# blue-yonder/tsfresh

Measured on AMD Instinct MI355X. Metric: series/sec (ComprehensiveFCParameters, len=1024), higher is better.
Workload: dtype f64; 1 GPU; 100000 series/GPU x len 1024 float32 i.i.d. N(0,1), ComprehensiveFCParameters (783 columns), inputs and outputs resident in HBM; n_series_per_gpu=100000, length=1024, n_cols=783, parallelism=ids1

## Files before the change

tsfresh_amd/csrc/fam_spectral.h:

```cpp
#ifndef TSFA_FAM_SPECTRAL_H
#define TSFA_FAM_SPECTRAL_H

#include "tsfa_common.h"

#define TSFA_TW_N 65536

TSFA_DEV bool is_pow2(int n) { return n > 0 && (n & (n - 1)) == 0; }

TSFA_DEV void blk_fft_stages_dit(const Blk &b, double *re, double *im, int M, const double *twc, const double *tws);

TSFA_DEV void blk_fft_pow2(const Blk &b, double *re, double *im, int M, const double *twc, const double *tws) {
    int logM = 0;
    while ((1 << logM) < M) ++logM;
    blk_sync();
    for (int i = b.tid; i < M; i += b.nt) {
#if TSFA_GPU
        const int j = (logM > 0) ? (int)(__builtin_bitreverse32((unsigned)i) >> (32 - logM)) : 0;
#else
        unsigned r = 0, x = (unsigned)i;
        for (int k = 0; k < logM; ++k) {
            r = (r << 1) | (x & 1u);
            x >>= 1;
        }
        const int j = (int)r;
#endif
        if (j > i) {
            const double tr = re[i], ti = im[i];
            re[i] = re[j];
            im[i] = im[j];
            re[j] = tr;
            im[j] = ti;
        }
    }
    blk_fft_stages_dit(b, re, im, M, twc, tws);
}

TSFA_DEV void blk_fft_stages_dit(const Blk &b, double *re, double *im, int M, const double *twc, const double *tws) {
    int logM = 0;
    while ((1 << logM) < M) ++logM;
    int st = 0;
    if (logM & 1) {
        blk_sync();
        for (int t = b.tid; t < (M >> 1); t += b.nt) {
            const int i0 = 2 * t, i1 = i0 + 1;
            const double wr = twc[0], wi = tws[0];
            const double xr = re[i1], xi = im[i1];
            const double tr = xr * wr - xi * wi;
            const double ti = xr * wi + xi * wr;
            const double ur = re[i0], ui = im[i0];
            re[i1] = ur - tr;
            im[i1] = ui - ti;
            re[i0] = ur + tr;
            im[i0] = ui + ti;
        }
        st = 1;
    }
    for (; st + 1 < logM; st += 2) {
        const int h = 1 << st;
        const int strideA = TSFA_TW_N / (2 * h), strideB = TSFA_TW_N / (4 * h);
        blk_sync();
        for (int t = b.tid; t < (M >> 2); t += b.nt) {
            const int grp = t >> st, k = t & (h - 1);
            const int i0 = grp * 4 * h + k, i1 = i0 + h, i2 = i0 + 2 * h, i3 = i0 + 3 * h;
            const double war = twc[k * strideA], wai = tws[k * strideA];
            const double wbr0 = twc[k * strideB], wbi0 = tws[k * strideB];
            const double wbr1 = twc[(k + h) * strideB], wbi1 = tws[(k + h) * strideB];
            const double x0r = re[i0], x0i = im[i0], x1r = re[i1], x1i = im[i1];
            const double x2r = re[i2], x2i = im[i2], x3r = re[i3], x3i = im[i3];
            double tr = x1r * war - x1i * wai, ti = x1r * wai + x1i * war;
            const double a1r = x0r - tr, a1i = x0i - ti, a0r = x0r + tr, a0i = x0i + ti;
            tr = x3r * war - x3i * wai;
            ti = x3r * wai + x3i * war;
            const double a3r = x2r - tr, a3i = x2i - ti, a2r = x2r + tr, a2i = x2i + ti;
            tr = a2r * wbr0 - a2i * wbi0;
            ti = a2r * wbi0 + a2i * wbr0;
            re[i2] = a0r - tr;
            im[i2] = a0i - ti;
            re[i0] = a0r + tr;
            im[i0] = a0i + ti;
            tr = a3r * wbr1 - a3i * wbi1;
            ti = a3r * wbi1 + a3i * wbr1;
            re[i3] = a1r - tr;
            im[i3] = a1i - ti;
            re[i1] = a1r + tr;
            im[i1] = a1i + ti;
        }
    }
    blk_sync();
}

TSFA_DEV void blk_fft_pow2_batch(const Blk &b, double *re, double *im, int M, int nb, const double *twc, const double *tws) {
    int logM = 0;
    while ((1 << logM) < M) ++logM;
    blk_sync();
    for (int ii = b.tid; ii < nb * M; ii += b.nt) {
        const int base = ii & ~(M - 1), i = ii & (M - 1);
#if TSFA_GPU
        const int j = (logM > 0) ? (int)(__builtin_bitreverse32((unsigned)i) >> (32 - logM)) : 0;
#else
        unsigned r = 0, x = (unsigned)i;
        for (int k = 0; k < logM; ++k) {
            r = (r << 1) | (x & 1u);
            x >>= 1;
        }
        const int j = (int)r;
#endif
        if (j > i) {
            const double tr = re[base + i], ti = im[base + i];
            re[base + i] = re[base + j];
            im[base + i] = im[base + j];
            re[base + j] = tr;
            im[base + j] = ti;
        }
    }
    int st = 0;
    if (logM & 1) {
        blk_sync();
        for (int t = b.tid; t < nb * (M >> 1); t += b.nt) {
            const int i0 = 2 * t, i1 = i0 + 1;
            const double wr = twc[0], wi = tws[0];
            const double xr = re[i1], xi = im[i1];
            const double tr = xr * wr - xi * wi;
            const double ti = xr * wi + xi * wr;
            const double ur = re[i0], ui = im[i0];
            re[i1] = ur - tr;
            im[i1] = ui - ti;
            re[i0] = ur + tr;
            im[i0] = ui + ti;
        }
        st = 1;
    }
    const int lq = logM - 2;
    for (; st + 1 < logM; st += 2) {
        const int h = 1 << st;
        const int strideA = TSFA_TW_N / (2 * h), strideB = TSFA_TW_N / (4 * h);
        blk_sync();
        for (int tt = b.tid; tt < nb * (M >> 2); tt += b.nt) {
            const int blk = tt >> lq, t = tt & ((M >> 2) - 1);
            const int grp = t >> st, k = t & (h - 1);
            const int i0 = blk * M + grp * 4 * h + k, i1 = i0 + h, i2 = i0 + 2 * h, i3 = i0 + 3 * h;
            const double war = twc[k * strideA], wai = tws[k * strideA];
            const double wbr0 = twc[k * strideB], wbi0 = tws[k * strideB];
            const double wbr1 = twc[(k + h) * strideB], wbi1 = tws[(k + h) * strideB];
            const double x0r = re[i0], x0i = im[i0], x1r = re[i1], x1i = im[i1];
            const double x2r = re[i2], x2i = im[i2], x3r = re[i3], x3i = im[i3];
            double tr = x1r * war - x1i * wai, ti = x1r * wai + x1i * war;
            const double a1r = x0r - tr, a1i = x0i - ti, a0r = x0r + tr, a0i = x0i + ti;
            tr = x3r * war - x3i * wai;
            ti = x3r * wai + x3i * war;
            const double a3r = x2r - tr, a3i = x2i - ti, a2r = x2r + tr, a2i = x2i + ti;
            tr = a2r * wbr0 - a2i * wbi0;
            ti = a2r * wbi0 + a2i * wbr0;
            re[i2] = a0r - tr;
            im[i2] = a0i - ti;
            re[i0] = a0r + tr;
            im[i0] = a0i + ti;
            tr = a3r * wbr1 - a3i * wbi1;
            ti = a3r * wbi1 + a3i * wbr1;
            re[i3] = a1r - tr;
            im[i3] = a1i - ti;
            re[i1] = a1r + tr;
            im[i1] = a1i + ti;
        }
    }
    blk_sync();
}

#define TSFA_GOERTZEL_MIN 257

template <class G>
TSFA_DEV void blk_rfft(const Blk &b, int n, G g, double *Xr, double *Xi, double *tc, double *ts,
                       const double *twc, const double *tws) {
    const int nh = n / 2;
    if (is_pow2(n) && n >= 4 && n <= TSFA_TW_N) {
        const int M = nh;
        blk_sync();
        for (int k = b.tid; k < M; k += b.nt) {
            Xr[k] = g(2 * k);
            Xi[k] = g(2 * k + 1);
        }
        blk_fft_pow2(b, Xr, Xi, M, twc, tws);
        const int stride = TSFA_TW_N / n;
        for (int k = b.tid; k <= M / 2; k += b.nt) {
            if (k == 0) {
                const double zr = Xr[0], zi = Xi[0];
                Xr[0] = zr + zi;
                Xi[0] = 0.0;
                Xr[M] = zr - zi;
                Xi[M] = 0.0;
            } else {
                const int k2 = M - k;
                const double ar = Xr[k], ai = Xi[k], br = Xr[k2], bi = Xi[k2];
                {
                    const double er = 0.5 * (ar + br), ei = 0.5 * (ai - bi);
                    const double orr = 0.5 * (ai + bi), oi = -0.5 * (ar - br);
                    const double wr = twc[k * stride], wi = tws[k * stride];
                    Xr[k] = er + (orr * wr - oi * wi);
                    Xi[k] = ei + (orr * wi + oi * wr);
                }
                if (k2 != k) {
                    const double er = 0.5 * (br + ar), ei = 0.5 * (bi - ai);
                    const double orr = 0.5 * (bi + ai), oi = -0.5 * (br - ar);
                    const double wr = twc[k2 * stride], wi = tws[k2 * stride];
                    Xr[k2] = er + (orr * wr - oi * wi);
                    Xi[k2] = ei + (orr * wi + oi * wr);
                }
            }
        }
        blk_sync();
        return;
    }
    double x_first;
    {
        double acc = 0.0;
        for (int j = b.tid; j < n; j += b.nt) acc += g(j);
        x_first = blk_sum(b, acc) / (double)n;
        if (!(x_first == x_first) || isinf(x_first)) x_first = 0.0;
    }
    if (n > 32768) {
        blk_sync();
        for (int k0 = 4 * b.tid; k0 <= nh; k0 += 4 * b.nt) {
            double kap[4], sg[4], sn[4], cs[4], s1[4], d1[4];
#pragma unroll
            for (int u = 0; u < 4; ++u) {
                double sh, ch;
                tsfa_sincospi(2.0 * (double)(k0 + u) / (double)n, &sn[u], &cs[u]);
                tsfa_sincospi((double)(k0 + u) / (double)n, &sh, &ch);
                const bool pos = cs[u] >= 0.0;
                kap[u] = pos ? -4.0 * sh * sh : 4.0 * ch * ch;
                sg[u] = pos ? 1.0 : -1.0;
                s1[u] = 0.0;
                d1[u] = 0.0;
            }
            for (int j = 0; j < n; ++j) {
                const double x = g(j) - x_first;
#pragma unroll
                for (int u = 0; u < 4; ++u) {
                    const double d = (x + kap[u] * s1[u]) + sg[u] * d1[u];
                    s1[u] = sg[u] * s1[u] + d;
                    d1[u] = d;
                }
            }
#pragma unroll
            for (int u = 0; u < 4; ++u) {
                const int k = k0 + u;
                if (k > nh) continue;
                Xr[k] = 0.5 * kap[u] * s1[u] + sg[u] * d1[u] + ((k == 0) ? (double)n * x_first : 0.0);
                Xi[k] = (k == 0 || 2 * k == n) ? 0.0 : s1[u] * sn[u];
            }
        }
        blk_sync();
        return;
    }
    if (n >= TSFA_GOERTZEL_MIN) {
        blk_sync();
        for (int k0 = 4 * b.tid; k0 <= nh; k0 += 4 * b.nt) {
            double c[4], sn[4], cs[4], s1[4], s2[4];
#pragma unroll
            for (int u = 0; u < 4; ++u) {
                tsfa_sincospi(2.0 * (double)(k0 + u) / (double)n, &sn[u], &cs[u]);
                c[u] = 2.0 * cs[u];
                s1[u] = 0.0;
                s2[u] = 0.0;
            }
            for (int j = 0; j < n; ++j) {
                const double x = g(j) - x_first;
#pragma unroll
                for (int u = 0; u < 4; ++u) {
                    const double s0 = (x + c[u] * s1[u]) - s2[u];
                    s2[u] = s1[u];
                    s1[u] = s0;
                }
            }
#pragma unroll
            for (int u = 0; u < 4; ++u) {
                const int k = k0 + u;
                if (k > nh) continue;
                Xr[k] = s1[u] * cs[u] - s2[u] + ((k == 0) ? (double)n * x_first : 0.0);
                Xi[k] = (k == 0 || 2 * k == n) ? 0.0 : s1[u] * sn[u];
            }
        }
        blk_sync();
        return;
    }
    blk_sync();
    for (int j = b.tid; j < n; j += b.nt) {
        double s, c;
        tsfa_sincospi(2.0 * (double)j / (double)n, &s, &c);
        tc[j] = c;
        ts[j] = -s;
    }
    blk_sync_all();
    for (int k = b.tid; k <= nh; k += b.nt) {
        double ar = 0.0, ai = 0.0;
        int idx = 0;
        for (int j = 0; j < n; ++j) {
            const double x = g(j) - x_first;
            ar += x * tc[idx];
            ai += x * ts[idx];
            idx += k;
            if (idx >= n) idx -= n;
        }
        if (k == 0 || (2 * k == n)) ai = 0.0;
        if (k == 0) ar += (double)n * x_first;
        Xr[k] = ar;
        Xi[k] = ai;
    }
    blk_sync();
}

#define TSFA_BLUESTEIN_MAXM 65536

TSFA_DEV int tsfa_bitrev(int i, int bits) {
#if TSFA_GPU
    return (bits > 0) ? (int)(__builtin_bitreverse32((unsigned)i) >> (32 - bits)) : 0;
#else
    unsigned r = 0, x = (unsigned)i;
    for (int k = 0; k < bits; ++k) { r = (r << 1) | (x & 1u); x >>= 1; }
    return (int)r;
#endif
}

TSFA_DEV void blk_fft_stages_dif(const Blk &b, double *re, double *im, int M, const double *twc, const double *tws) {
    int logM = 0;
    while ((1 << logM) < M) ++logM;
    int st = logM;
    for (; st >= 2; st -= 2) {
        const int h = 1 << (st - 2);
        const int strideA = TSFA_TW_N / (4 * h), strideB = TSFA_TW_N / (2 * h);
        blk_sync();
        for (int t = b.tid; t < (M >> 2); t += b.nt) {
            const int grp = t >> (st - 2), k = t & (h - 1);
            const int i0 = grp * 4 * h + k, i1 = i0 + h, i2 = i0 + 2 * h, i3 = i0 + 3 * h;
            const double wa0r = twc[k * strideA], wa0i = tws[k * strideA];
            const double wa1r = twc[(k + h) * strideA], wa1i = tws[(k + h) * strideA];
            const double wbr = twc[k * strideB], wbi = tws[k * strideB];
            const double x0r = re[i0], x0i = im[i0], x1r = re[i1], x1i = im[i1];
            const double x2r = re[i2], x2i = im[i2], x3r = re[i3], x3i = im[i3];
            const double a0r = x0r + x2r, a0i = x0i + x2i, d0r = x0r - x2r, d0i = x0i - x2i;
            const double a2r = d0r * wa0r - d0i * wa0i, a2i = d0r * wa0i + d0i * wa0r;
            const double a1r = x1r + x3r, a1i = x1i + x3i, d1r = x1r - x3r, d1i = x1i - x3i;
// ... 208 lines not shown
                Xi[N] = 0.0;
            } else {
                const int k2 = N - k;
                double ar, ai, br, bi;
                zbin(k, &ar, &ai);
                zbin(k2, &br, &bi);
                {
                    const double er = 0.5 * (ar + br), ei = 0.5 * (ai - bi);
                    const double orr = 0.5 * (ai + bi), oi = -0.5 * (ar - br);
                    double c, s;
                    unit(2 * k, &c, &s);
                    const double wr = c, wi = -s;
                    Xr[k] = er + (orr * wr - oi * wi);
                    Xi[k] = ei + (orr * wi + oi * wr);
                }
                if (k2 != k) {
                    const double er = 0.5 * (br + ar), ei = 0.5 * (bi - ai);
                    const double orr = 0.5 * (bi + ai), oi = -0.5 * (br - ar);
                    double c, s;
                    unit(2 * k2, &c, &s);
                    const double wr = c, wi = -s;
                    Xr[k2] = er + (orr * wr - oi * wi);
                    Xi[k2] = ei + (orr * wi + oi * wr);
                }
            }
        }
    }
    blk_sync();
}

template <class ST>
TSFA_DEV int blk_welch(const Blk &b, const ST *xs, int n, double *win, double *pxx, double *Xr, double *Xi,
                       double *tc, double *ts, const double *twc, const double *tws, int xcap = 0,
                       const double *hann256 = nullptr) {
    const int nper = (n < 256) ? n : 256;
    const int nover = nper / 2;
    const int step = nper - nover;
    const int nseg = (n - nover) / step;
    const int nf = nper / 2 + 1;
    blk_sync();
    double w2 = 0.0;
    for (int j = b.tid; j < nper; j += b.nt) {
        double wv;
        if (nper == 256 && hann256 != nullptr) wv = hann256[j];
        else {
            const double fac = np_linspace_at(-M_PI, M_PI, nper + 1, j);
            wv = (nper <= 1) ? 1.0 : (0.5 + 0.5 * cos(fac));
        }
        win[j] = wv;
        w2 += wv * wv;
    }
    for (int k = b.tid; k < nf; k += b.nt) pxx[k] = 0.0;
    w2 = blk_sum(b, w2);
    const double scale = 1.0 / w2;
    const int nbmax = (xcap / 128 < TSFA_RED_DOUBLES / 2) ? xcap / 128 : TSFA_RED_DOUBLES / 2;
    if (nper == 256 && nseg > 1 && nbmax >= 2) {
        const int M = 128;
        const int stride_tw = TSFA_TW_N / 256;
        for (int s0 = 0; s0 < nseg; s0 += nbmax) {
            const int nb = (nseg - s0 < nbmax) ? (nseg - s0) : nbmax;
            blk_sync();
#if TSFA_GPU
            {
                const int lane = b.tid & 63, wave = b.tid >> 6, nwav = (b.nt + 63) >> 6;
                for (int q = wave; q < nb; q += nwav) {
                    const XsView<ST> seg{xs + (s0 + q) * step};
                    double sm = 0.0;
                    for (int j = lane; j < nper; j += 64) sm += seg[j];
                    const double mu = wave_sum(sm) / (double)nper;
                    if (lane == 0) b.red[q] = mu;
                }
            }
#else
            for (int q = b.tid; q < nb; q += b.nt) {
                const XsView<ST> seg{xs + (s0 + q) * step};
                double sm = 0.0;
                for (int j = 0; j < nper; ++j) sm += seg[j];
                b.red[q] = sm / (double)nper;
            }
#endif
            blk_sync();
            for (int i = b.tid; i < nb * M; i += b.nt) {
                const int q = i >> 7, k = i & (M - 1);
                const XsView<ST> seg{xs + (s0 + q) * step};
                const double mu = b.red[q];
                Xr[i] = (seg[2 * k] - mu) * win[2 * k];
                Xi[i] = (seg[2 * k + 1] - mu) * win[2 * k + 1];
            }
            blk_fft_pow2_batch(b, Xr, Xi, M, nb, twc, tws);
            for (int i = b.tid; i < nb * (M / 2 + 1); i += b.nt) {
                const int q = i / (M / 2 + 1), k = i - q * (M / 2 + 1);
                double *zr = Xr + q * M, *zi = Xi + q * M;
                if (k == 0) {
                    const double a0 = zr[0], b0 = zi[0];
                    const double x0 = a0 + b0, xm = a0 - b0;
                    zr[0] = (x0 * x0 + 0.0 * 0.0) * scale;
                    zi[0] = (xm * xm + 0.0 * 0.0) * scale;
                } else {
                    const int k2 = M - k;
                    const double ar = zr[k], ai = zi[k], br = zr[k2], bi = zi[k2];
                    double pk, pk2 = 0.0;
                    {
                        const double er = 0.5 * (ar + br), ei = 0.5 * (ai - bi);
                        const double orr = 0.5 * (ai + bi), oi = -0.5 * (ar - br);
                        const double wr = twc[k * stride_tw], wi = tws[k * stride_tw];
                        const double xr = er + (orr * wr - oi * wi), xi = ei + (orr * wi + oi * wr);
                        pk = (xr * xr + xi * xi) * scale * 2.0;
                    }
                    if (k2 != k) {
                        const double er = 0.5 * (br + ar), ei = 0.5 * (bi - ai);
                        const double orr = 0.5 * (bi + ai), oi = -0.5 * (br - ar);
                        const double wr = twc[k2 * stride_tw], wi = tws[k2 * stride_tw];
                        const double xr = er + (orr * wr - oi * wi), xi = ei + (orr * wi + oi * wr);
                        pk2 = (xr * xr + xi * xi) * scale * 2.0;
                    }
                    zr[k] = pk;
                    if (k2 != k) zr[k2] = pk2;
                }
            }
            blk_sync();
            for (int k = b.tid; k < nf; k += b.nt) {
                double acc = pxx[k];
                for (int q = 0; q < nb; ++q) acc += (k < M) ? Xr[q * M + k] : Xi[q * M];
                pxx[k] = acc;
            }
            blk_sync();
        }
    } else
    for (int sgi = 0; sgi < nseg; ++sgi) {
        const XsView<ST> seg{xs + sgi * step};
        double sm = 0.0;
        for (int j = b.tid; j < nper; j += b.nt) sm += seg[j];
        const double mu = blk_sum(b, sm) / (double)nper;
        const double *wn = win;
        blk_rfft(b, nper, [=](int j) { return (seg[j] - mu) * wn[j]; }, Xr, Xi, tc, ts, twc, tws);
        for (int k = b.tid; k < nf; k += b.nt) {
            double pw = (Xr[k] * Xr[k] + Xi[k] * Xi[k]) * scale;
            const bool edge = (k == 0) || ((nper % 2 == 0) && (k == nf - 1));
            if (!edge) pw *= 2.0;
            pxx[k] += pw;
        }
        blk_sync();
    }
    if (nseg > 0)
        for (int k = b.tid; k < nf; k += b.nt) pxx[k] = pxx[k] / (double)nseg;
    blk_sync();
    return nf;
}

template <class ST, bool BL = true>
TSFA_DEV void fam_spectral_series(const Blk &b, const ST *xs_raw, int n, const TsfaSpec *specs, int nspecs,
                                  double *out_row, double *Xr, double *Xi, double *tc, double *ts, double *win,
                                  double *pxx, int *iw, const double *twc, const double *tws, int flags, int nlead,
                                  double *gs = nullptr, const double *hann256 = nullptr, double *chirp_tab = nullptr,
                                  int bl_min = TSFA_BLUESTEIN_PACK(TSFA_BLUESTEIN_MIN, TSFA_BLUESTEIN_MIN_EVEN)) {
    const XsView<ST> xs{xs_raw};
    const bool need_fft = (flags & 1) != 0, need_welch = (flags & 2) != 0;
    const int nf = n / 2 + 1;
    TSFA_TICKER(tk, 0);

    int npx = 0;
    double pmax = 0.0, pmin = 0.0;
    bool pnan = false;
    if (need_welch) {
        npx = blk_welch(b, xs_raw, n, win, pxx, Xr, Xi, tc, ts, twc, tws, (n / 2 + 2 > 260) ? n / 2 + 2 : 260, hann256);
        double mx = -TSFA_INF, mn = TSFA_INF, nn = 0.0;
        for (int k = b.tid; k < npx; k += b.nt) {
            mx = fmax(mx, pxx[k]);
            mn = fmin(mn, pxx[k]);
            nn += (pxx[k] != pxx[k]) ? 1.0 : 0.0;
        }
        pmax = blk_max(b, mx);
        pmin = blk_min(b, mn);
        pnan = blk_sum(b, nn) > 0.0;
    }
    TSFA_TICK(tk, b, 170);
    for (int s = 0; s < nlead; ++s) {
        const TsfaSpec sp = specs[s];
        double v = TSFA_NAN;
        if (sp.calc == TSFA_C_SPKT_WELCH_DENSITY) {
            const int c = (int)sp.p[0];
            v = (c >= 0 && c < npx) ? pxx[c] : TSFA_NAN;
        } else if (sp.calc == TSFA_C_FOURIER_ENTROPY) {
            const int bins = (int)sp.p[0];
            const double *px = pxx;
            const double pm = pmax;
            const double lo = pmin / pmax, hi = pmax / pmax;
            if (pnan || lo != lo || hi != hi || isinf(lo) || isinf(hi)) v = TSFA_NAN;
            else v = blk_binned_entropy(b, npx, [=](int i) { return px[i] / pm; }, bins, lo, hi, iw, 128);
        } else {
            continue;
        }
        if (b.tid == 0) out_row[sp.col] = v;
    }
    TSFA_TICK(tk, b, 171);
    if (!need_fft) return;

    if (BL && gs != nullptr && chirp_tab != nullptr && n >= ((n & 1) ? (bl_min & 0xFFFF) : (int)((unsigned)bl_min >> 16)) && !is_pow2(n) && bluestein_tiles_ok(n))
        blk_rfft_bluestein(b, n, [=](int j) { return xs[j]; }, Xr, Xi, gs, chirp_tab, twc, tws);
    else
        blk_rfft(b, n, [=](int j) { return xs[j]; }, Xr, Xi, tc, ts, twc, tws);
    TSFA_TICK(tk, b, 172);
    double s0 = 0.0, s1 = 0.0, s2 = 0.0, s3 = 0.0, s4 = 0.0;
    for (int k = b.tid; k < nf; k += b.nt) {
        const double a = hypot(Xr[k], Xi[k]);
        const double dk = (double)k;
        s0 += a;
        s1 += a * dk;
        s2 += a * (dk * dk);
        s3 += a * (dk * dk * dk);
        s4 += a * (dk * dk * dk * dk);
    }
    {
        double s5[5] = {s0, s1, s2, s3, s4};
        blk_sum_multi<5>(b, s5);
        s0 = s5[0]; s1 = s5[1]; s2 = s5[2]; s3 = s5[3]; s4 = s5[4];
    }
    const double m1 = s1 / s0, m2 = s2 / s0, m3 = s3 / s0, m4 = s4 / s0;
    const double var = m2 - m1 * m1;
    for (int s = nlead + b.tid; s < nspecs; s += b.nt) {
        const TsfaSpec sp = specs[s];
        double v = TSFA_NAN;
// ... 25 lines not shown
```

tsfresh_amd/csrc/tsfa_api.cpp:

```cpp
#include <hip/hip_runtime.h>

#include <stdio.h>
#include <stdlib.h>

#include <algorithm>
#include <string>
#include <vector>

#include "../../include/tsfresh_amd.h"
#include "tsfa_host_tables.h"
#include "tsfa_launch.h"
#include "fam_seq.h"
#include "tsfa_layout.h"

static thread_local std::string g_last_error;

static int fail(int code, const std::string &msg) {
    g_last_error = msg;
    return code;
}

int tsfa_fail(int code, const char *msg) { return fail(code, std::string(msg ? msg : "")); }
#define HIP_TRY(expr)                                                                                    \
    do {                                                                                                 \
// ... 538 lines not shown
                side_forked = true;
            }
            fst = plan->side;
            side_used = true;
        }
        const char *slot_name = (plan->stream_ok && (f == TSFA_FAM_SORT || (f == TSFA_FAM_BASIC && plan->fam_specs[TSFA_FAM_SORT].empty())))
                                    ? "k_stream" : fam_names[f];
        if (record(plan, fst, slot, slot_name, true)) return fail(TSFA_ERR_HIP, "event record failed");
        std::vector<TsfaLaunch> perm_launches;
        for (int g = sh.n_groups - 1; g >= 0; --g) {
            const int maxn = sh.g_maxn[g];
            const long long max_np2 = sh.g_np2[g];
            TsfaLaunch a;
            memset(&a, 0, sizeof a);
            a.fam = f;
            a.dtype = dtype;
            a.values = d_values;
            a.starts = d_starts;
            a.ends = d_ends;
            a.n_series = sh.g_count[g];
            a.sel = (sh.n_groups > 1) ? d_sel + sh.map.base[g] : nullptr;
            a.specs = plan->d_specs[f];
            a.nspecs = (int)plan->fam_specs[f].size();
            a.out = d_out;
            a.ld = ld;
            a.maxn = maxn;
            a.nt = (maxn <= 2048) ? 64 : 256;
            if (maxn > 2048) {
                static const int nt_8k[TSFA_N_FAMILIES] = {512, 512, 512, 512, 256, 1024, 256, 256};
                static const int nt_4k[TSFA_N_FAMILIES] = {256, 256, 256, 256, 256, 512, 256, 256};
                a.nt = (maxn > 4096) ? nt_8k[f] : nt_4k[f];
            }
            if (maxn <= 2048) {
                static const int pref[TSFA_N_FAMILIES] = {64, 128, 128, 64, 256, 256, 128, 64};
                const int cap = std::max(64, ((maxn / 4 + 63) / 64) * 64);
                a.nt = std::min(pref[f], cap);
            }
            if (TSFA_LAB_ONLY(plan->opt.nt[f] >= 64)) a.nt = plan->opt.nt[f];
            a.stream = fst;
            a.dectab = plan->d_dectab;
            a.times = d_times;
            a.twc = plan->d_twc;
            a.consts = plan->d_consts;
            a.tws = plan->d_tws;
            a.hint_a = plan->hints[f].a;
            a.hint_b = plan->hints[f].b;
            a.hint_c = plan->hints[f].c;
            a.hint_d = plan->hints[f].d;
            a.hint_e = plan->hints[f].e;
            a.alt = plan->hints[f].alt;
            a.cq = plan->hints[f].cq;
            if (f == TSFA_FAM_SPECTRAL && maxn > 2048 && !TSFA_LAB_ONLY(plan->opt.nt[f] >= 64)) a.nt = 512;
            int aux = 0;
            if (f == TSFA_FAM_TREND) aux = a.alt.small_w;
            if (f == TSFA_FAM_SPECTRAL) {
                a.dft_n = (int)std::min<long long>(max_np2, 256);
                aux = a.dft_n;
                int bl_odd = TSFA_BLUESTEIN_MIN, bl_even = TSFA_BLUESTEIN_MIN_EVEN;
                if (plan->opt.bluestein_min > 0) bl_odd = bl_even = std::min(std::max(plan->opt.bluestein_min, 17), 32767);
                a.bluestein_min = TSFA_BLUESTEIN_PACK(bl_odd, bl_even);
                if (max_np2 >= std::min(bl_odd, bl_even) && max_np2 <= 32768 && plan->opt.bluestein) {
                    long long M = 1;
                    while (M < 2 * max_np2 - 1) M <<= 1;
                    const size_t slot_bytes = (size_t)(4 * M) * sizeof(double);
                    int64_t slots = std::min<int64_t>(a.n_series, std::max<int64_t>((int64_t)((1ull << 30) / slot_bytes), 2048));
                    if (plan->opt.gscratch_slots > 0) slots = std::min<int64_t>(slots, plan->opt.gscratch_slots);
                    const size_t bytes = (size_t)slots * slot_bytes;
// ... 505 lines not shown
```

tsfresh_amd/csrc/tsfa_common.h:

```cpp
#ifndef TSFA_COMMON_H
#define TSFA_COMMON_H

#include <math.h>
#include <stdint.h>

#include "tsfa_specs.h"

#if defined(__HIPCC__)
#include <hip/hip_runtime.h>
#define TSFA_GPU 1
#define TSFA_DEV __device__ __forceinline__
#define TSFA_DEVN __device__ __noinline__
#define TSFA_MEM __device__ __forceinline__
#else
#define TSFA_GPU 0
#define TSFA_DEV static inline
#define TSFA_DEVN static
#define TSFA_MEM inline
#endif
#if defined(__HIP_DEVICE_COMPILE__)
#define TSFA_ASSUME_LDS(p) __builtin_assume(__builtin_amdgcn_is_shared((const void *)(p)))
#else
#define TSFA_ASSUME_LDS(p) ((void)0)
#endif
// ... 51 lines not shown
        if (tid == 0) tsfa_ticks_lds[base + id] += now - t;
        t = __builtin_readcyclecounter();
    }
};
#define TSFA_TICKER(name, base) Ticker name(base)
#define TSFA_TICK(name, b, id) name.mark((b).tid, id)
#define TSFA_TICKS_BEGIN()                                                                  \
    do {                                                                                    \
        for (int i_ = threadIdx.x; i_ < 256; i_ += blockDim.x) tsfa_ticks_lds[i_] = 0ull;   \
        __syncthreads();                                                                    \
    } while (0)
#define TSFA_TICKS_END()                                                                    \
    do {                                                                                    \
        __syncthreads();                                                                    \
        for (int i_ = threadIdx.x; i_ < 256; i_ += blockDim.x)                              \
            if (tsfa_ticks_lds[i_]) atomicAdd(&tsfa_ticks[i_], tsfa_ticks_lds[i_]);         \
    } while (0)
#else
#define TSFA_TICKER(name, base)
#define TSFA_TICK(name, b, id)
#define TSFA_TICKS_BEGIN()
#define TSFA_TICKS_END()
#endif

TSFA_DEV void blk_sync() {
#if TSFA_GPU
#if defined(TSFA_LONG)
    asm volatile("s_waitcnt vmcnt(0) lgkmcnt(0)" ::: "memory");
    __syncthreads();
#else
    asm volatile("s_waitcnt lgkmcnt(0)\n\ts_barrier" ::: "memory");
#endif
#endif
}
TSFA_DEV void blk_sync_all() {
#if TSFA_GPU
    asm volatile("s_waitcnt vmcnt(0) lgkmcnt(0)" ::: "memory");
    __syncthreads();
#endif
}

#if TSFA_GPU
template <int CTRL>
TSFA_DEV double dpp_mov_f64(double v) {
    union { double d; int i[2]; } a, r;
    a.d = v;
    r.i[0] = __builtin_amdgcn_update_dpp(a.i[0], a.i[0], CTRL, 0xf, 0xf, false);
    r.i[1] = __builtin_amdgcn_update_dpp(a.i[1], a.i[1], CTRL, 0xf, 0xf, false);
    return r.d;
}
TSFA_DEV double readlane_f64(double v, int lane) {
    union { double d; int i[2]; } a, r;
    a.d = v;
    r.i[0] = __builtin_amdgcn_readlane(a.i[0], lane);
    r.i[1] = __builtin_amdgcn_readlane(a.i[1], lane);
    return r.d;
}
#define TSFA_DPP_QUAD_XOR1 0xB1
#define TSFA_DPP_QUAD_XOR2 0x4E
#define TSFA_DPP_ROW_HALF_MIRROR 0x141
#define TSFA_DPP_ROW_MIRROR 0x140
TSFA_DEV double wave_sum(double v) {
    v += dpp_mov_f64<TSFA_DPP_QUAD_XOR1>(v);
    v += dpp_mov_f64<TSFA_DPP_QUAD_XOR2>(v);
    v += dpp_mov_f64<TSFA_DPP_ROW_HALF_MIRROR>(v);
    v += dpp_mov_f64<TSFA_DPP_ROW_MIRROR>(v);
// ... 1106 lines not shown
    if (i == div && num_edges > 1) return stop;
    const double delta = stop - start;
    const double step = delta / (double)div;
    if (step == 0.0) return ((double)i / (double)div) * delta + start;
    return (double)i * step + start;
}

template <bool RECIP, class BT, class G>
TSFA_DEV void binned_scatter(const BT &b, int m, G g, int bins, double first, double last, double norm, double inv_norm, double step,
                             bool flat, int c0, int cb, int *cnt) {
    for (int i = b.tid; i < m; i += b.nt) {
        const double v = g(i);
        if (!(v >= first && v <= last)) continue;
        const double fidx = RECIP ? ((v - first) * inv_norm) * (double)bins : ((v - first) / norm) * (double)bins;
        int idx = (fidx < 2147483000.0) ? (int)fidx : (bins - 1);
        if (idx >= bins) idx = bins - 1;
        if (idx < 0) idx = 0;
        const double e0 = flat ? np_linspace_at(first, last, bins + 1, idx) : ((idx == bins) ? last : (double)idx * step + first);
        if (v < e0) idx -= 1;
        if (idx != bins - 1) {
            const double e1 = flat ? np_linspace_at(first, last, bins + 1, idx + 1)
                                   : ((idx + 1 == bins) ? last : (double)(idx + 1) * step + first);
            if (v >= e1) idx += 1;
        }
        if (idx < c0 || idx >= c0 + cb) continue;
#if TSFA_GPU
        atomicAdd(&cnt[idx - c0], 1);
#else
        cnt[idx - c0] += 1;
#endif
    }
}

template <class BT, class G>
TSFA_DEV double blk_binned_entropy(const BT &b, int m, G g, int bins, double vmin, double vmax, int *cnt, int cap = 256) {
    double first = vmin, last = vmax;
    if (!(fabs(first) < TSFA_INF) || !(fabs(last) < TSFA_INF)) return TSFA_NAN;
    if (first == last) {
        first = first - 0.5;
        last = last + 0.5;
    }
    const double norm = last - first;
    const double inv_norm = 1.0 / norm;
    const bool recip = (inv_norm < TSFA_INF) && (inv_norm >= 2.2250738585072014e-308);
    const double delta = last - first, step = delta / (double)bins;
    const bool flat = (step == 0.0);
    {
        const double amax = fmax(fabs(first), fabs(last));
        if (!(step > 8.9e-16 * amax)) {
            unsigned stuck = 0;
            for (int k = b.tid; k < bins; k += b.nt)
                if (np_linspace_at(first, last, bins + 1, k) >= np_linspace_at(first, last, bins + 1, k + 1)) stuck = 1;
            if (blk_or16(b, stuck) != 0) return TSFA_NAN;
        }
    }
    double e = 0.0;
    for (int c0 = 0; c0 < bins; c0 += cap) {
        const int cb = (bins - c0 < cap) ? (bins - c0) : cap;
        blk_sync();
        for (int k = b.tid; k < cb; k += b.nt) cnt[k] = 0;
        blk_sync();
        if (recip) binned_scatter<true>(b, m, g, bins, first, last, norm, inv_norm, step, flat, c0, cb, cnt);
        else binned_scatter<false>(b, m, g, bins, first, last, norm, inv_norm, step, flat, c0, cb, cnt);
        blk_sync();
        for (int k = b.tid; k < cb; k += b.nt) {
            const int c = cnt[k];
            if (c > 0) {
                const double p = (double)c / (double)m;
                e += p * log(p);
            }
        }
    }
    e = blk_sum(b, e);
    return -e;
}

#endif
```

tsfresh_amd/csrc/tsfa_kernels.hip:

```cpp
#include <hip/hip_runtime.h>

#include "fam_ar.h"
#include "fam_ar_dd.h"
#include "fam_basic.h"
#include "fam_cwt.h"
#include "fam_entropy.h"
#include "fam_seq.h"
#include "fam_perm.h"
#include "fam_sort.h"
#include "fam_spectral.h"
#include "fam_general.h"
#include "tsfa_launch.h"
#include "tsfa_layout.h"

#include <algorithm>

#if defined(TSFA_LONG)
#define TSFA_GS_PARAMS , unsigned char *__restrict__ gsc, size_t gslot
#define TSFA_GS_ARGS , gsc, gslot
#define TSFA_SERIES_BEGIN                                                           \
    unsigned char *const tsfa_base = gsc + (size_t)blockIdx.x * gslot;             \
    for (int64_t wi_ = blockIdx.x; wi_ < n_series; wi_ += gridDim.x) {             \
        const int64_t sidx = sel ? (int64_t)sel[wi_] : wi_;
#define TSFA_SERIES_END \
// ... 216 lines not shown
                       const TsfaSpec *__restrict__ specs, int nspecs, double *__restrict__ out, int64_t ld, int maxn, int tau) {
    TSFA_SERIES_BEGIN
    const int64_t off = starts[sidx];
    const int n = (int)(ends[sidx] - off);
    PermLds L;
    L.carve(tsfa_base, maxn, blockDim.x, (int)sizeof(T), TSFA_PE_HIST_WORDS, TSFA_PE_LOGS + TSFA_PE_MAXD + 1);
    TSFA_TICKS_BEGIN();
    Blk b{(int)threadIdx.x, (int)blockDim.x, L.red, nullptr};
    T *xs = (T *)L.xs;
    {
        const T *__restrict__ g = values + off;
        for (int i = b.tid; i < n; i += b.nt) xs[i] = g[i];
        blk_sync();
    }
    fam_perm_series<T>(b, xs, n, specs, nspecs, out + sidx * ld, tau, L.iw, L.ltab);
    TSFA_TICKS_END();
    TSFA_SERIES_END
}
#endif

template <typename T, bool BL>
__global__ void __launch_bounds__(1024) k_spectral(const T *__restrict__ values, const int64_t *__restrict__ starts, const int64_t *__restrict__ ends, int64_t n_series, const int *__restrict__ sel,
                           const TsfaSpec *__restrict__ specs, int nspecs, double *__restrict__ out, int64_t ld,
                           int maxn, int dft_n, double *__restrict__ gscratch, int gscratch_n, int bl_min,
                           const double *__restrict__ twc, const double *__restrict__ tws, int hint_a, int hint_b,
                           const double *__restrict__ consts TSFA_GS_PARAMS) {
    TSFA_SERIES_BEGIN
    const int64_t off = starts[sidx];
    const int n = (int)(ends[sidx] - off);
    SpectralLds L;
    L.carve(tsfa_base, maxn, dft_n, (int)sizeof(T));
    TSFA_TICKS_BEGIN();
    Blk b{(int)threadIdx.x, (int)blockDim.x, L.red, nullptr};
    T *xs = (T *)L.xs;
    {
        const T *__restrict__ g = values + off;
        for (int i = b.tid; i < n; i += b.nt) xs[i] = g[i];
        blk_sync();
    }
    double *gs = gscratch ? gscratch + (size_t)blockIdx.x * (size_t)gscratch_n : nullptr;
    fam_spectral_series<T, BL>(b, xs, n, specs, nspecs, out + sidx * ld, L.Xr, L.Xi, L.tc, L.ts, L.win, L.pxx, L.iw, twc, tws,
                        hint_a, hint_b, gs, consts ? consts + TSFA_CONSTS_HANN : nullptr, L.chirp_tab(), bl_min);
    TSFA_TICKS_END();
    TSFA_SERIES_END
}

template <typename T>
__global__ void __launch_bounds__(1024) k_ar(const T *__restrict__ values, const int64_t *__restrict__ starts, const int64_t *__restrict__ ends, int64_t n_series, const int *__restrict__ sel,
                     const TsfaSpec *__restrict__ specs, int nspecs, double *__restrict__ out, int64_t ld, int maxn,
                     int P, int hint_acf, int hint_pacf, int hint_adf, int n_loop, long long *__restrict__ deg_list,
                     int *__restrict__ deg_count, const double *__restrict__ stats_in TSFA_GS_PARAMS) {
    TSFA_SERIES_BEGIN
    const int64_t off = starts[sidx];
    const int n = (int)(ends[sidx] - off);
    ArLds L;
    L.carve(tsfa_base, maxn, P, (int)sizeof(T), (int)blockDim.x);
    TSFA_TICKS_BEGIN();
    Blk b{(int)threadIdx.x, (int)blockDim.x, L.red, L.np};
    const T *g = values + off;
    const int flags = fam_ar_series<T>(b, [=](int i) { return (double)g[i]; }, n, specs, nspecs, out + sidx * ld,
                                       (void *)L.xc, L.aw, P, hint_acf, hint_pacf, hint_adf, n_loop,
                                       stats_in ? stats_in + sidx * TSFA_STATS_N : nullptr, L.part, L.part_doubles);
    if (flags && threadIdx.x == 0) deg_list[atomicAdd(deg_count, 1)] = ((long long)sidx << 2) | flags;
    TSFA_TICKS_END();
    TSFA_SERIES_END
}

#if !defined(TSFA_LONG)
__global__ void __launch_bounds__(64) k_langevin_dd(const double *__restrict__ pf_buf, const int *__restrict__ pf_count, int pf_slot, int pf_cap,
                     const TsfaSpec *__restrict__ specs, int nspecs, double *__restrict__ out, int64_t ld) {
    const int cnt = min(*pf_count, pf_cap);
    const int rmax = (pf_slot - TSFA_PF_HDR) / 2;
    for (int i = blockIdx.x * 64 + threadIdx.x; i < cnt; i += gridDim.x * 64) {
        const double *rec = pf_buf + (size_t)i * (size_t)pf_slot;
        const int64_t sidx = (int64_t)rec[0];
// ... 1040 lines not shown
```

tsfresh_amd/csrc/tsfa_layout.h:

```cpp
#ifndef TSFA_LAYOUT_H
#define TSFA_LAYOUT_H

#include <stddef.h>
#include <stdint.h>

#include "tsfa_common.h"
#include "fam_cwt.h"
#include "fam_seq.h"
#include "tsfa_entb_params.h"

#if defined(__HIPCC__)
#define TSFA_HD __host__ __device__ inline
#else
#define TSFA_HD inline
#endif

#define TSFA_LDS_LIMIT (160 * 1024)

struct LdsCarve {
    unsigned char *base;
    size_t off;
    template <class U>
    TSFA_HD U *take(size_t count) {
        off = (off + 15) & ~(size_t)15;
// ... 53 lines not shown
        cum = w;
        altc = (part & 2) ? c.take<double>(8 * 16) : nullptr;
        ctx = c.take<double>(32);
        iw = c.take<int>((part & 2) ? 16 * 6 * 2 : TSFA_ROW_BINS);
        return c.off;
    }
};

struct SortLds {
    double *red; NpScratch *np; void *xs; void *srt; double *w; int *iw; double *cq; TsfaSpec *stage; double *ctx;
    TSFA_HD size_t carve(unsigned char *base, int maxn, int nt, int xs_bytes = 8, int w_doubles = 1280) {
        (void)nt;
        LdsCarve c{base, 0};
        red = c.take<double>(TSFA_RED_DOUBLES);
        np = c.take<NpScratch>(1);
        xs = c.take<unsigned char>((size_t)maxn * xs_bytes);
        srt = c.take<unsigned char>((size_t)tsfa_pow2_ceil(maxn) * xs_bytes);
        w = c.take<double>(w_doubles);
        iw = (int *)w;
        cq = c.take<double>(5 * TSFA_CQ_MAX);
        ctx = c.take<double>(8);
#if defined(TSFA_SPEC_LDS)
        stage = c.take<TsfaSpec>(TSFA_SPEC_BATCH);
#else
        stage = nullptr;
#endif
        return c.off;
    }
};

struct SpectralLds {
    double *red; void *xs; double *Xr; double *Xi; double *tc; double *ts; double *win; double *pxx; int *iw;
    TSFA_HD size_t carve(unsigned char *base, int maxn, int dft_n, int xs_bytes = 8) {
        LdsCarve c{base, 0};
        red = c.take<double>(TSFA_RED_DOUBLES);
        xs = c.take<unsigned char>((size_t)maxn * xs_bytes);
        const int nx = (maxn / 2 + 2 > 260) ? maxn / 2 + 2 : 260;
        Xr = c.take<double>(nx);
        Xi = c.take<double>(nx);
        const int nd = (dft_n > 256) ? dft_n : (dft_n > 0 ? 256 : 2);
        tc = c.take<double>(nd);
        ts = c.take<double>(nd);
        win = c.take<double>(256);
        pxx = c.take<double>(dft_n > 0 ? 260 : 132);
        iw = (int *)(void *)win;
        has_chirp_tab = (nd == 256 && dft_n > 0);
        return c.off;
    }
    bool has_chirp_tab = false;
    TSFA_HD double *chirp_tab() const { return has_chirp_tab ? tc : nullptr; }
};

struct ArLds {
    double *red; NpScratch *np; double *xc; double *aw; double *part; int part_doubles;
    TSFA_HD static int scratch_doubles(int P) { return (P * (P - 1)) / 2 + 8 * P + 64 + 8 + 48 + 32; }
    TSFA_HD size_t carve(unsigned char *base, int maxn, int P, int xs_bytes = 8, int nt = 64) {
        LdsCarve c{base, 0};
        red = c.take<double>(TSFA_RED_DOUBLES);
        xc = (double *)(void *)c.take<unsigned char>((size_t)(maxn + 64 + 16) * xs_bytes);
        const size_t ab = (size_t)scratch_doubles(P) * sizeof(double);
        unsigned char *u = c.take<unsigned char>(ab > sizeof(NpScratch) ? ab : sizeof(NpScratch));
        aw = (double *)u;
        np = (NpScratch *)u;
        part_doubles = (nt > 64) ? 72 * ((nt + 63) / 64) : 0;
        part = part_doubles ? c.take<double>((size_t)part_doubles) : nullptr;
        return c.off;
    }
};

struct ArDdLds {
    double *red; double *scratch;
    TSFA_HD static int scratch_doubles(int P) { return 4 * P * P + 19 * (P + 1) + P + 10; }
    TSFA_HD size_t carve(unsigned char *base, int P) {
        LdsCarve c{base, 0};
        red = c.take<double>(TSFA_RED_DOUBLES);
        scratch = c.take<double>((size_t)scratch_doubles(P));
        return c.off;
    }
// ... 106 lines not shown
```

Measured before the change: 2.821 million series/sec.

## Use wave-level syncs, radix-8 FFT stages, and slimmer spectral LDS

Block barriers in the spectral FFT, Welch and entropy paths become wave-local waits when the block has at most 64 threads. The FFT stages are unified into one batched routine that adds radix-8 register passes, cutting the number of LDS round-trips and syncs. For short series, the spectral kernel stops staging the series and Hann window in LDS, reads them from global memory, and aliases the window and histogram scratch into the FFT buffers, shrinking the LDS footprint. The spectral family's preferred block size drops from 128 to 64 threads so the wave-sync path applies, trading intra-block parallelism for higher occupancy.

```diff
diff --git a/tsfresh_amd/csrc/fam_spectral.h b/tsfresh_amd/csrc/fam_spectral.h
--- a/tsfresh_amd/csrc/fam_spectral.h
+++ b/tsfresh_amd/csrc/fam_spectral.h
@@ -7,92 +7,16 @@
 
 TSFA_DEV bool is_pow2(int n) { return n > 0 && (n & (n - 1)) == 0; }
 
-TSFA_DEV void blk_fft_stages_dit(const Blk &b, double *re, double *im, int M, const double *twc, const double *tws);
-
-TSFA_DEV void blk_fft_pow2(const Blk &b, double *re, double *im, int M, const double *twc, const double *tws) {
+TSFA_DEV void fft_dit_stages(const Blk &b, double *re, double *im, int M, int nb, const double *twc, const double *tws);
+TSFA_DEV void blk_fft_stages_dit(const Blk &b, double *re, double *im, int M, const double *twc, const double *tws) {
+    fft_dit_stages(b, re, im, M, 1, twc, tws);
+}
+
+
+TSFA_DEV void fft_bitrev_blocks(const Blk &b, double *re, double *im, int M, int nb) {
     int logM = 0;
     while ((1 << logM) < M) ++logM;
-    blk_sync();
-    for (int i = b.tid; i < M; i += b.nt) {
-#if TSFA_GPU
-        const int j = (logM > 0) ? (int)(__builtin_bitreverse32((unsigned)i) >> (32 - logM)) : 0;
-#else
-        unsigned r = 0, x = (unsigned)i;
-        for (int k = 0; k < logM; ++k) {
-            r = (r << 1) | (x & 1u);
-            x >>= 1;
-        }
-        const int j = (int)r;
-#endif
-        if (j > i) {
-            const double tr = re[i], ti = im[i];
-            re[i] = re[j];
-            im[i] = im[j];
-            re[j] = tr;
-            im[j] = ti;
-        }
-    }
-    blk_fft_stages_dit(b, re, im, M, twc, tws);
-}
-
-TSFA_DEV void blk_fft_stages_dit(const Blk &b, double *re, double *im, int M, const double *twc, const double *tws) {
-    int logM = 0;
-    while ((1 << logM) < M) ++logM;
-    int st = 0;
-    if (logM & 1) {
-        blk_sync();
-        for (int t = b.tid; t < (M >> 1); t += b.nt) {
-            const int i0 = 2 * t, i1 = i0 + 1;
-            const double wr = twc[0], wi = tws[0];
-            const double xr = re[i1], xi = im[i1];
-            const double tr = xr * wr - xi * wi;
-            const double ti = xr * wi + xi * wr;
-            const double ur = re[i0], ui = im[i0];
-            re[i1] = ur - tr;
-            im[i1] = ui - ti;
-            re[i0] = ur + tr;
-            im[i0] = ui + ti;
-        }
-        st = 1;
-    }
-    for (; st + 1 < logM; st += 2) {
-        const int h = 1 << st;
-        const int strideA = TSFA_TW_N / (2 * h), strideB = TSFA_TW_N / (4 * h);
-        blk_sync();
-        for (int t = b.tid; t < (M >> 2); t += b.nt) {
-            const int grp = t >> st, k = t & (h - 1);
-            const int i0 = grp * 4 * h + k, i1 = i0 + h, i2 = i0 + 2 * h, i3 = i0 + 3 * h;
-            const double war = twc[k * strideA], wai = tws[k * strideA];
-            const double wbr0 = twc[k * strideB], wbi0 = tws[k * strideB];
-            const double wbr1 = twc[(k + h) * strideB], wbi1 = tws[(k + h) * strideB];
-            const double x0r = re[i0], x0i = im[i0], x1r = re[i1], x1i = im[i1];
-            const double x2r = re[i2], x2i = im[i2], x3r = re[i3], x3i = im[i3];
-            double tr = x1r * war - x1i * wai, ti = x1r * wai + x1i * war;
-            const double a1r = x0r - tr, a1i = x0i - ti, a0r = x0r + tr, a0i = x0i + ti;
-            tr = x3r * war - x3i * wai;
-            ti = x3r * wai + x3i * war;
-            const double a3r = x2r - tr, a3i = x2i - ti, a2r = x2r + tr, a2i = x2i + ti;
-            tr = a2r * wbr0 - a2i * wbi0;
-            ti = a2r * wbi0 + a2i * wbr0;
-            re[i2] = a0r - tr;
-            im[i2] = a0i - ti;
-            re[i0] = a0r + tr;
-            im[i0] = a0i + ti;
-            tr = a3r * wbr1 - a3i * wbi1;
-            ti = a3r * wbi1 + a3i * wbr1;
-            re[i3] = a1r - tr;
-            im[i3] = a1i - ti;
-            re[i1] = a1r + tr;
-            im[i1] = a1i + ti;
-        }
-    }
-    blk_sync();
-}
-
-TSFA_DEV void blk_fft_pow2_batch(const Blk &b, double *re, double *im, int M, int nb, const double *twc, const double *tws) {
-    int logM = 0;
-    while ((1 << logM) < M) ++logM;
-    blk_sync();
+    blk_sync_wave(b);
     for (int ii = b.tid; ii < nb * M; ii += b.nt) {
         const int base = ii & ~(M - 1), i = ii & (M - 1);
 #if TSFA_GPU
@@ -113,9 +37,26 @@
             im[base + j] = ti;
         }
     }
+}
+
+TSFA_DEV void blk_fft_pow2(const Blk &b, double *re, double *im, int M, const double *twc, const double *tws) {
+    fft_bitrev_blocks(b, re, im, M, 1);
+    fft_dit_stages(b, re, im, M, 1, twc, tws);
+}
+
+TSFA_DEV void blk_fft_pow2_batch(const Blk &b, double *re, double *im, int M, int nb, const double *twc, const double *tws) {
+    fft_bitrev_blocks(b, re, im, M, nb);
+    fft_dit_stages(b, re, im, M, nb, twc, tws);
+}
+
+TSFA_DEV void fft_dit_stages(const Blk &b, double *re, double *im, int M, int nb, const double *twc, const double *tws) {
+    int logM = 0;
+    while ((1 << logM) < M) ++logM;
+    const int n3 = (b.nt <= 64 && nb * (M >> 3) >= b.nt) ? logM / 3 : 0;
+    const int lead = logM - 3 * n3;
     int st = 0;
-    if (logM & 1) {
-        blk_sync();
+    if (lead & 1) {
+        blk_sync_wave(b);
         for (int t = b.tid; t < nb * (M >> 1); t += b.nt) {
             const int i0 = 2 * t, i1 = i0 + 1;
             const double wr = twc[0], wi = tws[0];
@@ -130,11 +71,11 @@
         }
         st = 1;
     }
-    const int lq = logM - 2;
-    for (; st + 1 < logM; st += 2) {
+    for (; st + 1 < lead; st += 2) {
         const int h = 1 << st;
+        const int lq = logM - 2;
         const int strideA = TSFA_TW_N / (2 * h), strideB = TSFA_TW_N / (4 * h);
-        blk_sync();
+        blk_sync_wave(b);
         for (int tt = b.tid; tt < nb * (M >> 2); tt += b.nt) {
             const int blk = tt >> lq, t = tt & ((M >> 2) - 1);
             const int grp = t >> st, k = t & (h - 1);
@@ -163,7 +104,44 @@
             im[i1] = a1i + ti;
         }
     }
-    blk_sync();
+    for (; st + 2 < logM; st += 3) {
+        const int h = 1 << st;
+        const int l8 = logM - 3;
+        blk_sync_wave(b);
+        for (int tt = b.tid; tt < nb * (M >> 3); tt += b.nt) {
+            const int blk = tt >> l8, t = tt & ((M >> 3) - 1);
+            const int grp = t >> st, k = t & (h - 1);
+            const int i0 = blk * M + grp * 8 * h + k;
+            double xr[8], xi[8];
+#pragma unroll
+            for (int q = 0; q < 8; ++q) {
+                xr[q] = re[i0 + q * h];
+                xi[q] = im[i0 + q * h];
+            }
+#pragma unroll
+            for (int s3 = 0; s3 < 3; ++s3) {
+                const int stride = TSFA_TW_N / ((2 * h) << s3);
+#pragma unroll
+                for (int q = 0; q < 8; ++q) {
+                    if (q & (1 << s3)) continue;
+                    const int q1 = q + (1 << s3);
+                    const int ti = (k + h * (q & ((1 << s3) - 1))) * stride;
+                    const double wr = twc[ti], wi = tws[ti];
+                    const double tr = xr[q1] * wr - xi[q1] * wi, tj = xr[q1] * wi + xi[q1] * wr;
+                    xr[q1] = xr[q] - tr;
+                    xi[q1] = xi[q] - tj;
+                    xr[q] = xr[q] + tr;
+                    xi[q] = xi[q] + tj;
+                }
+            }
+#pragma unroll
+            for (int q = 0; q < 8; ++q) {
+                re[i0 + q * h] = xr[q];
+                im[i0 + q * h] = xi[q];
+            }
+        }
+    }
+    blk_sync_wave(b);
 }
 
 #define TSFA_GOERTZEL_MIN 257
@@ -174,7 +152,7 @@
     const int nh = n / 2;
     if (is_pow2(n) && n >= 4 && n <= TSFA_TW_N) {
         const int M = nh;
-        blk_sync();
+        blk_sync_wave(b);
         for (int k = b.tid; k < M; k += b.nt) {
             Xr[k] = g(2 * k);
             Xi[k] = g(2 * k + 1);
@@ -207,7 +185,7 @@
                 }
             }
         }
-        blk_sync();
+        blk_sync_wave(b);
         return;
     }
     double x_first;
@@ -218,7 +196,7 @@
         if (!(x_first == x_first) || isinf(x_first)) x_first = 0.0;
     }
     if (n > 32768) {
-        blk_sync();
+        blk_sync_wave(b);
         for (int k0 = 4 * b.tid; k0 <= nh; k0 += 4 * b.nt) {
             double kap[4], sg[4], sn[4], cs[4], s1[4], d1[4];
 #pragma unroll
@@ -249,11 +227,11 @@
                 Xi[k] = (k == 0 || 2 * k == n) ? 0.0 : s1[u] * sn[u];
             }
         }
-        blk_sync();
+        blk_sync_wave(b);
         return;
     }
     if (n >= TSFA_GOERTZEL_MIN) {
-        blk_sync();
+        blk_sync_wave(b);
         for (int k0 = 4 * b.tid; k0 <= nh; k0 += 4 * b.nt) {
             double c[4], sn[4], cs[4], s1[4], s2[4];
 #pragma unroll
@@ -280,10 +258,10 @@
                 Xi[k] = (k == 0 || 2 * k == n) ? 0.0 : s1[u] * sn[u];
             }
         }
-        blk_sync();
+        blk_sync_wave(b);
         return;
     }
-    blk_sync();
+    blk_sync_wave(b);
     for (int j = b.tid; j < n; j += b.nt) {
         double s, c;
         tsfa_sincospi(2.0 * (double)j / (double)n, &s, &c);
@@ -306,7 +284,7 @@
         Xr[k] = ar;
         Xi[k] = ai;
     }
-    blk_sync();
+    blk_sync_wave(b);
 }
 
 #define TSFA_BLUESTEIN_MAXM 65536
@@ -581,22 +559,24 @@
 template <class ST>
 TSFA_DEV int blk_welch(const Blk &b, const ST *xs, int n, double *win, double *pxx, double *Xr, double *Xi,
                        double *tc, double *ts, const double *twc, const double *tws, int xcap = 0,
-                       const double *hann256 = nullptr) {
+                       const double *hann256 = nullptr, bool win_lds = true) {
     const int nper = (n < 256) ? n : 256;
     const int nover = nper / 2;
     const int step = nper - nover;
     const int nseg = (n - nover) / step;
     const int nf = nper / 2 + 1;
-    blk_sync();
+    blk_sync_wave(b);
     double w2 = 0.0;
+    const bool table = (nper == 256 && hann256 != nullptr);
+    const double *wn = (table && !win_lds) ? hann256 : win;
     for (int j = b.tid; j < nper; j += b.nt) {
         double wv;
-        if (nper == 256 && hann256 != nullptr) wv = hann256[j];
+        if (table) wv = hann256[j];
         else {
             const double fac = np_linspace_at(-M_PI, M_PI, nper + 1, j);
             wv = (nper <= 1) ? 1.0 : (0.5 + 0.5 * cos(fac));
         }
-        win[j] = wv;
+        if (!table || win_lds) win[j] = wv;
         w2 += wv * wv;
     }
     for (int k = b.tid; k < nf; k += b.nt) pxx[k] = 0.0;
@@ -608,7 +588,7 @@
         const int stride_tw = TSFA_TW_N / 256;
         for (int s0 = 0; s0 < nseg; s0 += nbmax) {
             const int nb = (nseg - s0 < nbmax) ? (nseg - s0) : nbmax;
-            blk_sync();
+            blk_sync_wave(b);
 #if TSFA_GPU
             {
                 const int lane = b.tid & 63, wave = b.tid >> 6, nwav = (b.nt + 63) >> 6;
@@ -628,13 +608,13 @@
                 b.red[q] = sm / (double)nper;
             }
 #endif
-            blk_sync();
+            blk_sync_wave(b);
             for (int i = b.tid; i < nb * M; i += b.nt) {
                 const int q = i >> 7, k = i & (M - 1);
                 const XsView<ST> seg{xs + (s0 + q) * step};
                 const double mu = b.red[q];
-                Xr[i] = (seg[2 * k] - mu) * win[2 * k];
-                Xi[i] = (seg[2 * k + 1] - mu) * win[2 * k + 1];
+                Xr[i] = (seg[2 * k] - mu) * wn[2 * k];
+                Xi[i] = (seg[2 * k + 1] - mu) * wn[2 * k + 1];
             }
             blk_fft_pow2_batch(b, Xr, Xi, M, nb, twc, tws);
             for (int i = b.tid; i < nb * (M / 2 + 1); i += b.nt) {
@@ -667,13 +647,13 @@
                     if (k2 != k) zr[k2] = pk2;
                 }
             }
-            blk_sync();
+            blk_sync_wave(b);
             for (int k = b.tid; k < nf; k += b.nt) {
                 double acc = pxx[k];
                 for (int q = 0; q < nb; ++q) acc += (k < M) ? Xr[q * M + k] : Xi[q * M];
                 pxx[k] = acc;
             }
-            blk_sync();
+            blk_sync_wave(b);
         }
     } else
     for (int sgi = 0; sgi < nseg; ++sgi) {
@@ -681,7 +661,6 @@
         double sm = 0.0;
         for (int j = b.tid; j < nper; j += b.nt) sm += seg[j];
         const double mu = blk_sum(b, sm) / (double)nper;
-        const double *wn = win;
         blk_rfft(b, nper, [=](int j) { return (seg[j] - mu) * wn[j]; }, Xr, Xi, tc, ts, twc, tws);
         for (int k = b.tid; k < nf; k += b.nt) {
             double pw = (Xr[k] * Xr[k] + Xi[k] * Xi[k]) * scale;
@@ -689,11 +668,11 @@
             if (!edge) pw *= 2.0;
             pxx[k] += pw;
         }
-        blk_sync();
+        blk_sync_wave(b);
     }
     if (nseg > 0)
         for (int k = b.tid; k < nf; k += b.nt) pxx[k] = pxx[k] / (double)nseg;
-    blk_sync();
+    blk_sync_wave(b);
     return nf;
 }
 
@@ -702,7 +681,8 @@
                                   double *out_row, double *Xr, double *Xi, double *tc, double *ts, double *win,
                                   double *pxx, int *iw, const double *twc, const double *tws, int flags, int nlead,
                                   double *gs = nullptr, const double *hann256 = nullptr, double *chirp_tab = nullptr,
-                                  int bl_min = TSFA_BLUESTEIN_PACK(TSFA_BLUESTEIN_MIN, TSFA_BLUESTEIN_MIN_EVEN)) {
+                                  int bl_min = TSFA_BLUESTEIN_PACK(TSFA_BLUESTEIN_MIN, TSFA_BLUESTEIN_MIN_EVEN),
+                                  bool win_lds = true) {
     const XsView<ST> xs{xs_raw};
     const bool need_fft = (flags & 1) != 0, need_welch = (flags & 2) != 0;
     const int nf = n / 2 + 1;
@@ -712,7 +692,8 @@
     double pmax = 0.0, pmin = 0.0;
     bool pnan = false;
     if (need_welch) {
-        npx = blk_welch(b, xs_raw, n, win, pxx, Xr, Xi, tc, ts, twc, tws, (n / 2 + 2 > 260) ? n / 2 + 2 : 260, hann256);
+        npx = blk_welch(b, xs_raw, n, win, pxx, Xr, Xi, tc, ts, twc, tws, (n / 2 + 2 > 260) ? n / 2 + 2 : 260, hann256,
+                        win_lds);
         double mx = -TSFA_INF, mn = TSFA_INF, nn = 0.0;
         for (int k = b.tid; k < npx; k += b.nt) {
             mx = fmax(mx, pxx[k]);
@@ -736,7 +717,7 @@
             const double pm = pmax;
             const double lo = pmin / pmax, hi = pmax / pmax;
             if (pnan || lo != lo || hi != hi || isinf(lo) || isinf(hi)) v = TSFA_NAN;
-            else v = blk_binned_entropy(b, npx, [=](int i) { return px[i] / pm; }, bins, lo, hi, iw, 128);
+            else v = blk_binned_entropy<true>(b, npx, [=](int i) { return px[i] / pm; }, bins, lo, hi, iw, 128);
         } else {
             continue;
         }
diff --git a/tsfresh_amd/csrc/tsfa_api.cpp b/tsfresh_amd/csrc/tsfa_api.cpp
--- a/tsfresh_amd/csrc/tsfa_api.cpp
+++ b/tsfresh_amd/csrc/tsfa_api.cpp
@@ -594,7 +594,7 @@
                 a.nt = (maxn > 4096) ? nt_8k[f] : nt_4k[f];
             }
             if (maxn <= 2048) {
-                static const int pref[TSFA_N_FAMILIES] = {64, 128, 128, 64, 256, 256, 128, 64};
+                static const int pref[TSFA_N_FAMILIES] = {64, 128, 64, 64, 256, 256, 128, 64};
                 const int cap = std::max(64, ((maxn / 4 + 63) / 64) * 64);
                 a.nt = std::min(pref[f], cap);
             }
diff --git a/tsfresh_amd/csrc/tsfa_common.h b/tsfresh_amd/csrc/tsfa_common.h
--- a/tsfresh_amd/csrc/tsfa_common.h
+++ b/tsfresh_amd/csrc/tsfa_common.h
@@ -107,6 +107,16 @@
     asm volatile("s_waitcnt lgkmcnt(0)\n\ts_barrier" ::: "memory");
 #endif
 #endif
+}
+TSFA_DEV void blk_sync_wave(const Blk &b) {
+#if TSFA_GPU && !defined(TSFA_LONG)
+    if (b.nt <= 64) {
+        asm volatile("s_waitcnt lgkmcnt(0)" ::: "memory");
+        return;
+    }
+#endif
+    (void)b;
+    blk_sync();
 }
 TSFA_DEV void blk_sync_all() {
 #if TSFA_GPU
@@ -1279,8 +1289,12 @@
     }
 }
 
-template <class BT, class G>
+template <bool WAVE_SYNC = false, class BT, class G>
 TSFA_DEV double blk_binned_entropy(const BT &b, int m, G g, int bins, double vmin, double vmax, int *cnt, int cap = 256) {
+    auto sync = [&]() {
+        if (WAVE_SYNC) blk_sync_wave(b);
+        else blk_sync();
+    };
     double first = vmin, last = vmax;
     if (!(fabs(first) < TSFA_INF) || !(fabs(last) < TSFA_INF)) return TSFA_NAN;
     if (first == last) {
@@ -1304,12 +1318,12 @@
     double e = 0.0;
     for (int c0 = 0; c0 < bins; c0 += cap) {
         const int cb = (bins - c0 < cap) ? (bins - c0) : cap;
-        blk_sync();
+        sync();
         for (int k = b.tid; k < cb; k += b.nt) cnt[k] = 0;
-        blk_sync();
+        sync();
         if (recip) binned_scatter<true>(b, m, g, bins, first, last, norm, inv_norm, step, flat, c0, cb, cnt);
         else binned_scatter<false>(b, m, g, bins, first, last, norm, inv_norm, step, flat, c0, cb, cnt);
-        blk_sync();
+        sync();
         for (int k = b.tid; k < cb; k += b.nt) {
             const int c = cnt[k];
             if (c > 0) {
diff --git a/tsfresh_amd/csrc/tsfa_kernels.hip b/tsfresh_amd/csrc/tsfa_kernels.hip
--- a/tsfresh_amd/csrc/tsfa_kernels.hip
+++ b/tsfresh_amd/csrc/tsfa_kernels.hip
@@ -272,15 +272,17 @@
     L.carve(tsfa_base, maxn, dft_n, (int)sizeof(T));
     TSFA_TICKS_BEGIN();
     Blk b{(int)threadIdx.x, (int)blockDim.x, L.red, nullptr};
-    T *xs = (T *)L.xs;
-    {
-        const T *__restrict__ g = values + off;
-        for (int i = b.tid; i < n; i += b.nt) xs[i] = g[i];
+    const T *xs = values + off;
+    if (L.xs != nullptr) {
+        T *xl = (T *)L.xs;
+        for (int i = b.tid; i < n; i += b.nt) xl[i] = xs[i];
         blk_sync();
+        xs = xl;
     }
     double *gs = gscratch ? gscratch + (size_t)blockIdx.x * (size_t)gscratch_n : nullptr;
     fam_spectral_series<T, BL>(b, xs, n, specs, nspecs, out + sidx * ld, L.Xr, L.Xi, L.tc, L.ts, L.win, L.pxx, L.iw, twc, tws,
-                        hint_a, hint_b, gs, consts ? consts + TSFA_CONSTS_HANN : nullptr, L.chirp_tab(), bl_min);
+                        hint_a, hint_b, gs, consts ? consts + TSFA_CONSTS_HANN : nullptr, L.chirp_tab(), bl_min,
+                        L.xs != nullptr);
     TSFA_TICKS_END();
     TSFA_SERIES_END
 }
diff --git a/tsfresh_amd/csrc/tsfa_layout.h b/tsfresh_amd/csrc/tsfa_layout.h
--- a/tsfresh_amd/csrc/tsfa_layout.h
+++ b/tsfresh_amd/csrc/tsfa_layout.h
@@ -109,18 +109,22 @@
 struct SpectralLds {
     double *red; void *xs; double *Xr; double *Xi; double *tc; double *ts; double *win; double *pxx; int *iw;
     TSFA_HD size_t carve(unsigned char *base, int maxn, int dft_n, int xs_bytes = 8) {
-        LdsCarve c{base, 0};
-        red = c.take<double>(TSFA_RED_DOUBLES);
-        xs = c.take<unsigned char>((size_t)maxn * xs_bytes);
+        const bool ln = maxn <= 2048 && dft_n == 0 && carve_as(nullptr, maxn, dft_n, xs_bytes, false) > 10240;
+        return carve_as(base, maxn, dft_n, xs_bytes, ln);
+    }
+    TSFA_HD size_t carve_as(unsigned char *base, int maxn, int dft_n, int xs_bytes, bool ln) {
+        LdsCarve c{base, 0};
+        red = c.take<double>(TSFA_RED_DOUBLES);
+        xs = ln ? nullptr : c.take<unsigned char>((size_t)maxn * xs_bytes);
         const int nx = (maxn / 2 + 2 > 260) ? maxn / 2 + 2 : 260;
         Xr = c.take<double>(nx);
         Xi = c.take<double>(nx);
         const int nd = (dft_n > 256) ? dft_n : (dft_n > 0 ? 256 : 2);
         tc = c.take<double>(nd);
         ts = c.take<double>(nd);
-        win = c.take<double>(256);
+        win = ln ? Xr + 130 : c.take<double>(256);
         pxx = c.take<double>(dft_n > 0 ? 260 : 132);
-        iw = (int *)(void *)win;
+        iw = ln ? (int *)(void *)Xi : (int *)(void *)win;
         has_chirp_tab = (nd == 256 && dft_n > 0);
         return c.off;
     }
```

Measured after the change: 2.831 million series/sec (median of 6 runs). About the same (+0.4%).
